# jinryan/RangeCLIP

Hardware: NVIDIA B200
Metric: pixel_text_infonce_fwd_bwd_throughput (higher is better)
Workload: dtype bf16

## Files before the change

rangeclip_b200/csrc/infonce_ts.cu:

```cuda
#include "infonce_pair.cuh"

namespace rc {
using namespace umma;

namespace ts {
using namespace cta_pair;

constexpr int kThreads = 640;
constexpr int kXStages = 6;
constexpr int kTStages = 3;
constexpr int kEpiBufs = 4;
constexpr int kEpiAhead = 2;
constexpr int kEpiBufBytes = 2048;
constexpr int kTmemCols = 512;
constexpr int kSlotCols = 256;
constexpr int kColAcc = 128, kAccCols = 64;
constexpr int kDxLead = 2;
constexpr int kRegsCtl = 48, kRegsSoftmax = 120;

struct __align__(8) Bars {
  uint64_t xf[kXStages];
  uint64_t xfull[kXStages], xempty[kXStages];
  uint64_t tfull[kTStages], tempty[kTStages];
  uint64_t s_full[2], p_full[2];
  uint64_t acc_full[2][2], acc_empty[2][2];
  uint64_t sc_full[4];
  uint64_t ebar[8][kEpiBufs];
  uint32_t tmem_base, pad;
};

constexpr int kScaleBufs = 4;
constexpr int kOffT = kXStages * kStageBytes;
constexpr int kOffEpi = kOffT + kTStages * kStageBytes;
constexpr int kOffScale = kOffEpi + 8 * kEpiBufs * kEpiBufBytes;
constexpr int kOffXch = kOffScale + kScaleBufs * 128 * 4;
constexpr int kOffPart = kOffXch + 2 * 4 * 2 * 128 * 4;
constexpr int kOffAcc = kOffPart + 8 * 128 * 4;
constexpr int kOffBars = kOffAcc + 3 * 128 * 4;
constexpr int kSmemBytes = kOffBars + (int)sizeof(Bars);
static_assert(kSmemBytes <= 232448, "shared-memory budget of one SM (227 KB)");

struct Params : Tiling {};

template <int R, bool kKB>
__global__ void __cluster_dims__(2, 1, 1) __launch_bounds__(kThreads, 1)
infonce_ts_kernel(const __grid_constant__ CUtensorMap map_x_s,
                  const __grid_constant__ CUtensorMap map_t,
                  const __grid_constant__ CUtensorMap map_tt,
                  const __grid_constant__ CUtensorMap map_xe,
                  const __grid_constant__ CUtensorMap map_dx,
                  const Params prm) {
  extern __shared__ __align__(1024) uint8_t smem[];
  Bars* bars = reinterpret_cast<Bars*>(smem + kOffBars);
  float* sc_s = reinterpret_cast<float*>(smem + kOffScale);
  const int warp = threadIdx.x >> 5, lane = threadIdx.x & 31;
  const uint32_t rank = cluster_ctarank();
  const bool leader_cta = rank == 0;
  const int n_dchunks = prm.D / 64;
  const int n_blk = prm.D / 64;
  const int n_kchunks = prm.Kp / 64;
  const int n_clusters = gridDim.x / 2;
  const int cluster_id = blockIdx.x / 2;
  const int my_pairs = cluster_id < prm.n_pairs ? (prm.n_pairs - cluster_id + n_clusters - 1) / n_clusters : 0;

  if (threadIdx.x == 0) {
    tma_prefetch_desc(&map_x_s); tma_prefetch_desc(&map_t); tma_prefetch_desc(&map_tt);
    tma_prefetch_desc(&map_xe); tma_prefetch_desc(&map_dx);
    for (int i = 0; i < kXStages; ++i) { mbar_init(&bars->xf[i], 1); mbar_init(&bars->xfull[i], 2); mbar_init(&bars->xempty[i], 9); }
    for (int i = 0; i < kTStages; ++i) { mbar_init(&bars->tfull[i], 1); mbar_init(&bars->tempty[i], 1); }
    for (int sl = 0; sl < 2; ++sl) {
      mbar_init(&bars->s_full[sl], 1); mbar_init(&bars->p_full[sl], 16);
      for (int ab = 0; ab < 2; ++ab) { mbar_init(&bars->acc_full[sl][ab], 1); mbar_init(&bars->acc_empty[sl][ab], 16); }
    }
    for (int i = 0; i < kScaleBufs; ++i) mbar_init(&bars->sc_full[i], 4);
    for (int i = 0; i < 8; ++i)
      for (int j = 0; j < kEpiBufs; ++j) mbar_init(&bars->ebar[i][j], 1);
    fence_barrier_init();
  }
  if (warp == 2) tmem_alloc_2sm<kTmemCols>(&bars->tmem_base);
  tc_fence_before();
  cluster_sync();
  tc_fence_after();
  const uint32_t tmem = bars->tmem_base;
#ifdef RC_TIMING
  long long wt[16];
#pragma unroll
  for (int i = 0; i < 16; ++i) wt[i] = 0;
  const long long t_start = clock64();
#endif
  const uint32_t idesc_s = make_idesc_bf16(256, prm.Kp,  1,  0);
  const uint32_t idesc_d = make_idesc_bf16(256, kAccCols, 0, 0);
  auto pair_of = [&](int l) -> int { return cluster_id + l * n_clusters; };

  if (warp < 4) {
    asm volatile("setmaxnreg.dec.sync.aligned.u32 %0;" ::"n"(kRegsCtl));
    if (warp == 0 && lane == 0) {
      uint32_t it = 0;
      auto load_s = [&](int l) {
        load_text_s<kTStages>(prm, &map_t, smem + kOffT, bars->tfull, bars->tempty, it, 0, n_dchunks,
                              text_row0<kKB>(prm, pair_of(l)), rank RC_WT);
      };
      auto load_dx = [&](int l, int b0, int b1) {
        const int koff = text_row0<kKB>(prm, pair_of(l));
        for (int blk = b0; blk < b1; ++blk, ++it) {
          const int st = it % kTStages;
          RC_WAIT(mbar_wait, &bars->tempty[st], ((it / kTStages) & 1) ^ 1, 2);
          if ((prm.ablate & 256) && it >= (uint32_t)kTStages) {
            if (leader_cta) mbar_arrive(&bars->tfull[st]);
            continue;
          }
          if (leader_cta) mbar_arrive_expect_tx(&bars->tfull[st], 2 * n_kchunks * 4096);
          for (int kc = 0; kc < n_kchunks; ++kc)
            tma_load_2d_2sm(smem + kOffT + st * kStageBytes + kc * 4096, &map_tt, &bars->tfull[st], koff + kc * 64,
                            blk * 64 + (int)rank * 32);
        }
      };
      if (my_pairs > 0) load_s(0);
      for (int l = 0; l < my_pairs; ++l) {
        load_dx(l, 0, kDxLead);
        if (l + 1 < my_pairs) load_s(l + 1);
        load_dx(l, kDxLead, n_blk);
      }
    } else if (warp == 3 && lane == 0) {
      uint32_t xit = 0;
      const uint64_t pol_keep = l2_policy_evict_last();
      for (int l = 0; l < my_pairs; ++l)
        load_x_tile<kXStages, kKB, true>(prm, &map_x_s, smem, bars->xf, bars->xempty, xit, 2 * pair_of(l) + (int)rank, n_dchunks,
                                         pol_keep, 3 RC_WT);
    } else if (warp == 1 && leader_cta) {
      uint32_t it = 0, xit = 0;
      uint32_t acc_par = 0;
      const uint32_t smem_base = smem_u32(smem);
      const uint64_t dsc_x = desc_mnmajor_sw128(0, 8192);
      const uint64_t dsc_k = desc_kmajor_sw128(0);
      auto wait_acc_free = [&](int sl, int ab, int tag) {
        RC_WAIT(mbar_wait, &bars->acc_empty[sl][ab], ((acc_par >> (2 * sl + ab)) & 1u) ^ 1u, tag);
      };
      auto issue_s = [&](int l) {
        const int sl = l & 1;
        const uint32_t s_tmem = tmem + sl * kSlotCols;
        wait_acc_free(sl, 0, 7);
        wait_acc_free(sl, 1, 7);
        tc_fence_after();
        RC_EV(l, 0);
        for (int c = 0; c < n_dchunks; ++c, ++it, ++xit) {
          const int sa = xit % kXStages, sb_ = it % kTStages;
          RC_WAIT(mbar_wait, &bars->xfull[sa], (xit / kXStages) & 1, 5);
          RC_WAIT(mbar_wait, &bars->tfull[sb_], (it / kTStages) & 1, 6);
          tc_fence_after();
          const uint64_t xa = dsc_x + ((smem_base + sa * kStageBytes) >> 4);
          const uint64_t tb = dsc_k + ((smem_base + kOffT + sb_ * kStageBytes) >> 4);
          if (elect_one()) {
#pragma unroll
            for (int ks = 0; ks < 4; ++ks)
              mma_bf16_ss_2sm(s_tmem, xa + ((ks * 2048) >> 4), tb + ((ks * 32) >> 4), idesc_s, (c | ks) != 0);
            mma_commit_2sm(&bars->xempty[sa]);
            mma_commit_2sm(&bars->tempty[sb_]);
            if (c + 1 == n_dchunks) mma_commit_2sm(&bars->s_full[sl]);
          }
          __syncwarp();
        }
        RC_EV(l, 1);
      };
      auto issue_dx = [&](int l, int b0, int b1) {
        const int sl = l & 1;
        const uint32_t base = tmem + sl * kSlotCols;
        if (b0 == 0) {
          RC_WAIT(mbar_wait, &bars->p_full[sl], (l >> 1) & 1, 9);
          tc_fence_after();
          RC_EV(l, 2);
        }
        for (int blk = b0; blk < b1; ++blk, ++it) {
          const int ab = blk & 1;
          wait_acc_free(sl, ab, 4);
          if (blk < 8) RC_EV(l, 3 + blk);
          const int st = it % kTStages;
          RC_WAIT(mbar_wait, &bars->tfull[st], (it / kTStages) & 1, 8);
          tc_fence_after();
          const uint64_t sb = dsc_k + ((smem_base + kOffT + st * kStageBytes) >> 4);
          const uint32_t dcol = base + kColAcc + ab * kAccCols;
          if (elect_one()) {
            for (int kc = 0; kc < n_kchunks; ++kc) {
#pragma unroll
              for (int ks = 0; ks < 4; ++ks)
                mma_bf16_ts_2sm(dcol, base + (kc * 4 + ks) * 8, sb + ((kc * 4096 + ks * 32) >> 4), idesc_d, (kc | ks) != 0);
            }
            mma_commit_2sm(&bars->tempty[st]);
            mma_commit_2sm(&bars->acc_full[sl][ab]);
          }
          __syncwarp();
          acc_par ^= 1u << (2 * sl + ab);
        }
        if (b1 == n_blk) RC_EV(l, 11);
      };
      if (my_pairs > 0) issue_s(0);
      for (int l = 0; l < my_pairs; ++l) {
        issue_dx(l, 0, kDxLead);
        if (l + 1 < my_pairs) issue_s(l + 1);
        issue_dx(l, kDxLead, n_blk);
      }
    } else if (warp == 2 && lane == 0) {
      uint32_t xit = 0;
      for (int l = 0; l < my_pairs; ++l) relay_x_tile<kXStages, false>(n_dchunks, bars->xf, bars->xfull, xit, leader_cta, 10 RC_WT);
    }
  } else if (warp < 12) {
    asm volatile("setmaxnreg.inc.sync.aligned.u32 %0;" ::"n"(kRegsSoftmax));
    const int half = warp >= 8 ? 1 : 0;
    const int row = (warp & 3) * 32 + lane;
    const int Kh = prm.Kp >> 1;
    const int cb = half * Kh;
    const uint32_t lane_base = tmem + ((uint32_t)((warp & 3) * 32) << 16);
    float* xch_base = reinterpret_cast<float*>(smem + kOffXch);
    float* acc_s = reinterpret_cast<float*>(smem + kOffAcc) + row;
    if (half == 0) acc_s[0] = acc_s[128] = acc_s[256] = 0.f;
    float gscale, inv_wsum;
    grad_scales(prm, gscale, inv_wsum);
    const float coefb = gscale * inv_wsum;
    float nx_ok, nx_w;
    int nx_y;
    load_pixel_scalars<R>(prm, 0 < my_pairs, 2 * pair_of(0) + (int)rank, row, nx_ok, nx_w, nx_y);
    float* part_s = reinterpret_cast<float*>(smem + kOffPart);
    int ng, nr;
    norm_coords(ng, nr);
    uint32_t nit = 0;
    const bool use_bound = prm.inv_tau * (2.02f * kLog2e) < 100.f;
    const float ml_bound = prm.inv_tau * (1.01f * kLog2e);
    for (int l = 0; l < my_pairs; ++l) {
      const int sl = l & 1;
      const int tile = 2 * pair_of(l) + (int)rank;
      const bool tile_ok = tile < prm.n_tiles;
      const int b = tile_ok ? div_tiles(prm, tile) : 0;
      const int px = tile_ok ? (tile - b * prm.tiles_per_img) * kTilePx + row : 0;
      const bool valid = tile_ok && px < prm.HW;
      const int64_t m = (int64_t)b * prm.HW + px;
      const int Kt = (kKB && prm.kb > 0) ? min(256, prm.K - 256 * b) : prm.K;
      const float ok = nx_ok;
      const bool px_ok = ok != 0.f;
      const int yi = nx_y;
      const float wi = (R == 1 && (yi >= 0 || (kKB && prm.keep_w))) ? nx_w : 0.f;
      load_pixel_scalars<R>(prm, l + 1 < my_pairs, 2 * pair_of(l + 1) + (int)rank, row, nx_ok, nx_w, nx_y);
      float* xch = xch_base + (l & 1) * (4 * 2 * 128);
      const uint32_t trow = lane_base + sl * kSlotCols + cb;
      RC_T0(tnorm);
      const float inv_n_tile = norm_tile<kXStages>(smem, bars->xf, bars->xempty, nit, n_dchunks, part_s, warp, lane, row, ng, nr, false,
                                                   11 RC_WT);
      RC_TACC(1, tnorm);
      if (warp == 4) RC_EV(l, 12);
      const float inv_n = px_ok ? inv_n_tile : 0.f;
      const float zs = inv_n * prm.inv_tau;
      const float zl = zs * kLog2e;
      RC_WAIT(mbar_wait, &bars->s_full[sl], (l >> 1) & 1, 12);
      tc_fence_after();
      if (warp == 4) RC_EV(l, 13);
      RC_T0(texp);
      const float ml = use_bound ? ml_bound : row_max(trow, Kt, cb, Kh, xch, half, row, zl);
      uint32_t pk[64];
      float sy[R];
      float sum, sez;
      exp_pass<R>(trow, cb, Kh, Kt, yi, zl, ml, pk, sy, sum, sez);
      int yj[R];
      float wj[R];
      bool mine[R];
      float wtot, tz;
      gather_targets<R>(prm, yi, wi, ok, m, cb, Kh, sy, yj, wj, mine, wtot, tz);
      post_sums(xch, half, row, sum, sez, tz);
      RC_TACC(2, texp);
      if (warp == 4) RC_EV(l, 14);
      tc_fence_before();
      RC_T0(txch);
      named_bar_sync(2, 256);
      RC_TACC(13, txch);
      tc_fence_after();
      RC_T0(tpst);
      add_peer_sums(xch, half, row, sum, sez, tz);
      const float lse = row_lse<kKB>(prm, valid, px, m, half, ml, wtot, tz, zs, sum, acc_s[0], acc_s[128]);
      const float coef = coefb * wtot;
      const float inv_sum = 1.f / sum;
      const float rsv = p_scale(inv_n, prm.inv_tau, coef, inv_sum);
      if (half == 0) {
        const float cj = proj_coef(coef, coefb, sez, tz, zs, inv_sum);
        sc_s[(l & (kScaleBufs - 1)) * 128 + row] = -(inv_n * inv_n * cj);
        acc_s[256] -= cj;
        __syncwarp();
        if (lane == 0) mbar_arrive(&bars->sc_full[l & (kScaleBufs - 1)]);
      }
      {
        const uint32_t prow = lane_base + sl * kSlotCols + (cb >> 1);
        const uint32_t rs2 = pack_bf16x2(rsv, rsv);
        uint32_t g16[R];
        int grel[R];
#pragma unroll
        for (int j = 0; j < R; ++j) {
          grel[j] = -1;
          g16[j] = 0;
          if (mine[j]) {
            const float gv = target_g<R>(j, sy, yj, wj, wtot, sum, zl, ml, rsv);
            grel[j] = yj[j] - cb;
            g16[j] = (uint32_t)__bfloat16_as_ushort(__float2bfloat16_rn(gv));
          }
        }
#pragma unroll
        for (int c = 0; c < 4; ++c) {
          if (c * 32 < Kh) {
            uint32_t v[16];
#pragma unroll
            for (int i = 0; i < 16; ++i) v[i] = bf2_mul(pk[c * 16 + i], rs2);
#pragma unroll
            for (int j = 0; j < R; ++j) {
              if (grel[j] >= 0 && (grel[j] >> 5) == c) {
                const int jj = (grel[j] >> 1) & 15;
                const bool hi = grel[j] & 1;
#pragma unroll
                for (int i = 0; i < 16; ++i)
                  if (i == jj) v[i] = hi ? ((v[i] & 0xffffu) | (g16[j] << 16)) : ((v[i] & 0xffff0000u) | g16[j]);
              }
            }
            tmem_st_32x16(prow + c * 16, v);
          }
        }
        tmem_st_wait();
        tc_fence_before();
        arrive_leader_warp(leader_cta, &bars->p_full[sl]);
      }
      RC_TACC(3, tpst);
      if (warp == 4) RC_EV(l, 15);
      if (half == 0 && valid && prm.lse && !(kKB && prm.lse_in != nullptr)) prm.lse[m] = lse;
    }
    if (half == 0) add_sums<true>(prm, lane, acc_s[0], acc_s[128], acc_s[256]);
  } else {
    const int ew = warp - 12;
    const int q = warp & 3, h = ew >> 2;
    uint8_t* ebuf = smem + kOffEpi + ew * (kEpiBufs * kEpiBufBytes);
    uint64_t* ebar = &bars->ebar[ew][0];
    const int total = my_pairs * n_blk;
    const uint64_t pol_first = l2_policy_evict_first();
    struct Cursor { int l, u, px, bo, bx; };
    auto cursor_pair = [&](Cursor& cu) {
      int b, px0;
      tile_coords(prm, 2 * pair_of(cu.l) + (int)rank, b, px0);
      cu.px = px0 + q * 32;
      cu.bo = b;
      cu.bx = (kKB && prm.kb > 0) ? (b < prm.B ? 0 : 1) : b;
    };
    auto cursor_next = [&](Cursor& cu) {
      if (++cu.u == n_blk) { cu.u = 0; ++cu.l; cursor_pair(cu); }
    };
    Cursor cs{0, 0, 0, 0, 0}, cr{0, 0, 0, 0, 0};
    cursor_pair(cs);
    cursor_pair(cr);
    int s_req = 0;
    auto request_x = [&]() {
      const int bi = s_req % kEpiBufs;
      if (prm.ablate & 1) {
        mbar_arrive(&ebar[bi]);
        return;
      }
      mbar_arrive_expect_tx(&ebar[bi], kEpiBufBytes);
      tma_load_3d_hint(ebuf + bi * kEpiBufBytes, &map_xe, &ebar[bi], cr.px, cr.u * 64 + h * 32, cr.bx, pol_first);
    };
    for (; s_req < kEpiAhead && s_req < total; ++s_req) {
      if (lane == 0) request_x();
      cursor_next(cr);
    }
    const uint32_t moff = (uint32_t)((lane & 7) * 64 + ((((lane >> 3) ^ ((lane >> 1) & 3)) & 3) << 4));
    int s = 0;
    uint32_t acc_par = 0;
    for (int l = 0; l < my_pairs; ++l) {
      const int sl = l & 1;
      RC_WAIT(mbar_wait, &bars->sc_full[l & (kScaleBufs - 1)], (l >> 2) & 1, 14);
      uint32_t ncs2[4];
#pragma unroll
      for (int pb = 0; pb < 4; ++pb) {
        const float v = sc_s[(l & (kScaleBufs - 1)) * 128 + q * 32 + pb * 8 + (lane >> 2)];
        ncs2[pb] = pack_bf16x2(v, v);
      }
      const uint32_t tacc = tmem + ((uint32_t)(q * 32) << 16) + sl * kSlotCols + kColAcc + h * 32;
      for (int blk = 0; blk < n_blk; ++blk, ++s) {
        const int ab = blk & 1;
        RC_WAIT(mbar_wait, &bars->acc_full[sl][ab], (acc_par >> (2 * sl + ab)) & 1u, 15);
        acc_par ^= 1u << (2 * sl + ab);
        tc_fence_after();
        if (warp == 12 && blk < 8) RC_EV(l, 20 + 2 * blk);
        RC_T0(tld);
        uint32_t pa[4][4];
        {
          uint32_t r[16];
          tmem_ld_16x256b_x4(tacc + ab * kAccCols, r);
          tmem_ld_wait();
#pragma unroll
          for (int g = 0; g < 4; ++g) {
            pa[g][0] = pack_bf16x2(__uint_as_float(r[4 * g]), __uint_as_float(r[4 * g + 1]));
            pa[g][1] = pack_bf16x2(__uint_as_float(r[4 * g + 2]), __uint_as_float(r[4 * g + 3]));
          }
          tmem_ld_16x256b_x4(tacc + ab * kAccCols + (16u << 16), r);
          tmem_ld_wait();
#pragma unroll
          for (int g = 0; g < 4; ++g) {
            pa[g][2] = pack_bf16x2(__uint_as_float(r[4 * g]), __uint_as_float(r[4 * g + 1]));
            pa[g][3] = pack_bf16x2(__uint_as_float(r[4 * g + 2]), __uint_as_float(r[4 * g + 3]));
          }
        }
        tc_fence_before();
        arrive_leader_warp(leader_cta, &bars->acc_empty[sl][ab]);
        RC_TACC(3, tld);
        const int bi = s % kEpiBufs;
        RC_WAIT(mbar_wait, &ebar[bi], (s / kEpiBufs) & 1, 4);
        RC_T0(tmath);
        const uint32_t bx0 = smem_u32(ebuf + bi * kEpiBufBytes) + moff;
        uint32_t xm[4][4];
#pragma unroll
        for (int g = 0; g < 4; ++g) ldmatrix_x4_trans(bx0 + g * 512, xm[g]);
#pragma unroll
        for (int g = 0; g < 4; ++g) {
#pragma unroll
          for (int pb = 0; pb < 4; ++pb) xm[g][pb] = bf2_fma(ncs2[pb], xm[g][pb], pa[g][pb]);
          stmatrix_x4_trans(bx0 + g * 512, xm[g]);
        }
        fence_proxy_async_smem();
        __syncwarp();
        RC_TACC(2, tmath);
        if (lane == 0) {
          if (!(prm.ablate & 2)) {
            if (kKB && prm.acc_dx) tma_reduce_add_3d(&map_dx, ebuf + bi * kEpiBufBytes, cs.px, cs.u * 64 + h * 32, cs.bo);
            else tma_store_3d_hint(&map_dx, ebuf + bi * kEpiBufBytes, cs.px, cs.u * 64 + h * 32, cs.bo, pol_first);
            tma_store_commit();
          }
          if (s_req < total) {
            RC_T0(tsw);
            asm volatile("cp.async.bulk.wait_group.read %0;" ::"n"(kEpiBufs - kEpiAhead) : "memory");
            RC_TACC(5, tsw);
            request_x();
          }
        }
        cursor_next(cs);
        if (s_req < total) { cursor_next(cr); ++s_req; }
        __syncwarp();
        if (warp == 12 && blk < 8) RC_EV(l, 21 + 2 * blk);
      }
    }
    if (lane == 0) tma_store_wait_all0();
  }
#ifdef RC_TIMING
  if (prm.dbg != nullptr && blockIdx.x < 2 && lane == 0 && (warp <= 1 || warp == 3 || warp == 4 || warp == 12)) {
    wt[0] = clock64() - t_start;
    const int role = warp == 0 ? 0 : (warp == 1 ? 1 : (warp == 4 ? 2 : (warp == 12 ? 3 : 4)));
#pragma unroll
    for (int i = 0; i < 16; ++i) prm.dbg[(blockIdx.x * 5 + role) * 16 + i] = wt[i];
  }
#endif
  tc_fence_before();
  cluster_sync();
  if (warp == 2) {
    tc_fence_after();
    tmem_dealloc_2sm<kTmemCols>(tmem);
  }
}

}

int launch_infonce_ts(const InfoncePairArgs& a, cudaStream_t s) {
  using namespace ts;
  CUtensorMap m_xs, m_t, m_tt, m_xe, m_dx;
  int rcode;
  if ((rcode = make_operand_maps(a, 32, {"ts map_x_s", "ts map_t", "ts map_tt"}, &m_xs, &m_t, &m_tt))) return rcode;
  if ((rcode = make_xmap(&m_xe, a.xsrc, a, a.kb > 0 ? 1 : a.B, 32, 32, "ts map_xe"))) return rcode;
  if ((rcode = make_xmap(&m_dx, a.dx, a, a.B, 32, 32, "ts map_dx"))) return rcode;
  Params prm;
  int grid = 0;
  if ((rcode = fill_tiling(prm, a, &grid))) return rcode;
  auto launch = [&](auto kernel) -> int {
    cudaError_t e = cudaFuncSetAttribute(kernel, cudaFuncAttributeMaxDynamicSharedMemorySize, kSmemBytes);
    if (e != cudaSuccess) return fail(RC_ERR_CUDA, "rc_infonce_bf16(ts): smem opt-in: %s", cudaGetErrorString(e));
    kernel<<<grid, kThreads, kSmemBytes, s>>>(m_xs, m_t, m_tt, m_xe, m_dx, prm);
    return check_launch("rc_infonce_bf16(ts)");
  };
  if (a.rep == 4) return launch(infonce_ts_kernel<4, false>);
  if (launch_kblocked(a)) return launch(infonce_ts_kernel<1, true>);
  return launch(infonce_ts_kernel<1, false>);
}

}
```

rangeclip_b200/csrc/umma.cuh:

```cuda
#pragma once
#include <cuda.h>
#include <cuda_runtime.h>
#include <stdint.h>
#include <stdio.h>

namespace rc {
namespace umma {

__device__ __forceinline__ uint32_t smem_u32(const void* p) {
  return (uint32_t)__cvta_generic_to_shared(p);
}

__device__ __forceinline__ void mbar_init(uint64_t* bar, uint32_t count) {
  asm volatile("mbarrier.init.shared::cta.b64 [%0], %1;" ::"r"(smem_u32(bar)), "r"(count) : "memory");
}
__device__ __forceinline__ void fence_barrier_init() {
  asm volatile("fence.mbarrier_init.release.cluster;" ::: "memory");
}
__device__ __forceinline__ void mbar_arrive(uint64_t* bar) {
  asm volatile("mbarrier.arrive.shared::cta.b64 _, [%0];" ::"r"(smem_u32(bar)) : "memory");
}
__device__ __forceinline__ void mbar_arrive_n(uint64_t* bar, uint32_t count) {
  asm volatile("mbarrier.arrive.shared::cta.b64 _, [%0], %1;" ::"r"(smem_u32(bar)), "r"(count) : "memory");
}
__device__ __forceinline__ void mbar_arrive_expect_tx(uint64_t* bar, uint32_t bytes) {
  asm volatile("mbarrier.arrive.expect_tx.shared::cta.b64 _, [%0], %1;" ::"r"(smem_u32(bar)), "r"(bytes) : "memory");
}
constexpr uint32_t kSuspendHintNs = 200000u;
__device__ __forceinline__ bool mbar_try_wait(uint64_t* bar, uint32_t parity) {
  uint32_t ok;
  asm volatile(
      "{\n\t.reg .pred p;\n\t"
      "mbarrier.try_wait.parity.shared::cta.b64 p, [%1], %2, %3;\n\t"
      "selp.u32 %0, 1, 0, p;\n\t}"
      : "=r"(ok)
      : "r"(smem_u32(bar)), "r"(parity), "r"(kSuspendHintNs)
      : "memory");
  return ok != 0;
}
__device__ __forceinline__ void mbar_wait(uint64_t* bar, uint32_t parity, int tag) {
#ifdef RC_BRINGUP
  if (mbar_try_wait(bar, parity)) return;
  const long long t0 = clock64();
  while (!mbar_try_wait(bar, parity)) {
    if (clock64() - t0 > 4000000000LL) {
      printf("rangeclip_b200: mbarrier timeout tag=%d block=%d thread=%d parity=%u\n", tag, (int)blockIdx.x,
             (int)threadIdx.x, parity);
      __trap();
    }
  }
#else
  (void)tag;
  while (!mbar_try_wait(bar, parity)) {}
#endif
}

__device__ __forceinline__ void fence_proxy_async_smem() {
  asm volatile("fence.proxy.async.shared::cta;" ::: "memory");
}
__device__ __forceinline__ void tc_fence_before() { asm volatile("tcgen05.fence::before_thread_sync;" ::: "memory"); }
__device__ __forceinline__ void tc_fence_after() { asm volatile("tcgen05.fence::after_thread_sync;" ::: "memory"); }
__device__ __forceinline__ void named_bar_sync(int id, int threads) {
  asm volatile("bar.sync %0, %1;" ::"r"(id), "r"(threads) : "memory");
}
__device__ __forceinline__ bool elect_one() {
  uint32_t pred;
  asm volatile(
      "{\n\t.reg .pred p;\n\t"
      "elect.sync _|p, 0xffffffff;\n\t"
      "selp.u32 %0, 1, 0, p;\n\t}"
      : "=r"(pred));
  return pred != 0;
}

__device__ __forceinline__ void tma_prefetch_desc(const CUtensorMap* m) {
  asm volatile("prefetch.tensormap [%0];" ::"l"(reinterpret_cast<uint64_t>(m)) : "memory");
}
__device__ __forceinline__ void tma_load_2d(void* dst, const CUtensorMap* m, uint64_t* bar, int c0, int c1) {
  asm volatile(
      "cp.async.bulk.tensor.2d.shared::cluster.global.mbarrier::complete_tx::bytes [%0], [%1, {%3, %4}], [%2];" ::"r"(
          smem_u32(dst)),
      "l"(reinterpret_cast<uint64_t>(m)), "r"(smem_u32(bar)), "r"(c0), "r"(c1)
      : "memory");
}
__device__ __forceinline__ void tma_load_3d(void* dst, const CUtensorMap* m, uint64_t* bar, int c0, int c1, int c2) {
  asm volatile(
      "cp.async.bulk.tensor.3d.shared::cluster.global.mbarrier::complete_tx::bytes [%0], [%1, {%3, %4, %5}], [%2];" ::"r"(
          smem_u32(dst)),
      "l"(reinterpret_cast<uint64_t>(m)), "r"(smem_u32(bar)), "r"(c0), "r"(c1), "r"(c2)
      : "memory");
}
__device__ __forceinline__ void tma_load_3d_hint(void* dst, const CUtensorMap* m, uint64_t* bar, int c0, int c1, int c2, uint64_t pol);
__device__ __forceinline__ uint64_t l2_policy_evict_first() {
  uint64_t p;
  asm volatile("createpolicy.fractional.L2::evict_first.b64 %0, 1.0;" : "=l"(p));
  return p;
}
__device__ __forceinline__ uint64_t l2_policy_evict_last() {
  uint64_t p;
  asm volatile("createpolicy.fractional.L2::evict_last.b64 %0, 1.0;" : "=l"(p));
  return p;
}
__device__ __forceinline__ void tma_load_3d_hint(void* dst, const CUtensorMap* m, uint64_t* bar, int c0, int c1, int c2, uint64_t pol) {
  asm volatile(
      "cp.async.bulk.tensor.3d.shared::cluster.global.mbarrier::complete_tx::bytes.L2::cache_hint [%0], [%1, {%3, %4, %5}], [%2], %6;" ::"r"(
          smem_u32(dst)),
      "l"(reinterpret_cast<uint64_t>(m)), "r"(smem_u32(bar)), "r"(c0), "r"(c1), "r"(c2), "l"(pol)
      : "memory");
}
__device__ __forceinline__ void tma_load_3d_2sm_hint(void* dst, const CUtensorMap* m, uint64_t* bar, int c0, int c1, int c2,
                                                     uint64_t pol) {
  asm volatile(
      "cp.async.bulk.tensor.3d.cta_group::2.shared::cluster.global.mbarrier::complete_tx::bytes.L2::cache_hint [%0], [%1, {%3, %4, %5}], [%2], %6;" ::"r"(
          smem_u32(dst)),
      "l"(reinterpret_cast<uint64_t>(m)), "r"(smem_u32(bar) & 0xFEFFFFFFu), "r"(c0), "r"(c1), "r"(c2), "l"(pol)
      : "memory");
}
__device__ __forceinline__ void tma_store_3d_hint(const CUtensorMap* m, const void* src, int c0, int c1, int c2, uint64_t pol) {
  asm volatile("cp.async.bulk.tensor.3d.global.shared::cta.bulk_group.L2::cache_hint [%0, {%2, %3, %4}], [%1], %5;" ::"l"(
                   reinterpret_cast<uint64_t>(m)),
               "r"(smem_u32(src)), "r"(c0), "r"(c1), "r"(c2), "l"(pol)
               : "memory");
}
__device__ __forceinline__ void tma_reduce_add_3d(const CUtensorMap* m, const void* src, int c0, int c1, int c2) {
  asm volatile("cp.reduce.async.bulk.tensor.3d.global.shared::cta.add.tile.bulk_group [%0, {%2, %3, %4}], [%1];" ::"l"(
                   reinterpret_cast<uint64_t>(m)),
               "r"(smem_u32(src)), "r"(c0), "r"(c1), "r"(c2)
               : "memory");
}
__device__ __forceinline__ void tma_prefetch_3d(const CUtensorMap* m, int c0, int c1, int c2) {
  asm volatile("cp.async.bulk.prefetch.tensor.3d.L2.global.tile [%0, {%1, %2, %3}];" ::"l"(reinterpret_cast<uint64_t>(m)), "r"(c0),
               "r"(c1), "r"(c2)
               : "memory");
}
__device__ __forceinline__ void tma_store_3d(const CUtensorMap* m, const void* src, int c0, int c1, int c2) {
  asm volatile("cp.async.bulk.tensor.3d.global.shared::cta.bulk_group [%0, {%2, %3, %4}], [%1];" ::"l"(
                   reinterpret_cast<uint64_t>(m)),
               "r"(smem_u32(src)), "r"(c0), "r"(c1), "r"(c2)
               : "memory");
}
__device__ __forceinline__ void tma_store_commit() { asm volatile("cp.async.bulk.commit_group;" ::: "memory"); }
__device__ __forceinline__ void tma_store_wait_read0() { asm volatile("cp.async.bulk.wait_group.read 0;" ::: "memory"); }
__device__ __forceinline__ void tma_store_wait_all0() { asm volatile("cp.async.bulk.wait_group 0;" ::: "memory"); }
__device__ __forceinline__ void tma_store_wait_read0_keep1() { asm volatile("cp.async.bulk.wait_group.read 1;" ::: "memory"); }

template <int kCols>
__device__ __forceinline__ void tmem_alloc(uint32_t* dst_smem) {
  asm volatile("tcgen05.alloc.cta_group::1.sync.aligned.shared::cta.b32 [%0], %1;" ::"r"(smem_u32(dst_smem)), "n"(kCols)
               : "memory");
  asm volatile("tcgen05.relinquish_alloc_permit.cta_group::1.sync.aligned;" ::: "memory");
}
template <int kCols>
__device__ __forceinline__ void tmem_dealloc(uint32_t taddr) {
  asm volatile("tcgen05.dealloc.cta_group::1.sync.aligned.b32 %0, %1;" ::"r"(taddr), "n"(kCols) : "memory");
}
__device__ __forceinline__ void tmem_ld_32x32(uint32_t taddr, uint32_t (&r)[32]) {
  asm volatile(
      "tcgen05.ld.sync.aligned.32x32b.x32.b32 "
      "{%0, %1, %2, %3, %4, %5, %6, %7, %8, %9, %10, %11, %12, %13, %14, %15, "
      "%16, %17, %18, %19, %20, %21, %22, %23, %24, %25, %26, %27, %28, %29, %30, %31}, [%32];"
      : "=r"(r[0]), "=r"(r[1]), "=r"(r[2]), "=r"(r[3]), "=r"(r[4]), "=r"(r[5]), "=r"(r[6]), "=r"(r[7]), "=r"(r[8]),
        "=r"(r[9]), "=r"(r[10]), "=r"(r[11]), "=r"(r[12]), "=r"(r[13]), "=r"(r[14]), "=r"(r[15]), "=r"(r[16]),
        "=r"(r[17]), "=r"(r[18]), "=r"(r[19]), "=r"(r[20]), "=r"(r[21]), "=r"(r[22]), "=r"(r[23]), "=r"(r[24]),
        "=r"(r[25]), "=r"(r[26]), "=r"(r[27]), "=r"(r[28]), "=r"(r[29]), "=r"(r[30]), "=r"(r[31])
      : "r"(taddr)
      : "memory");
}
__device__ __forceinline__ void tmem_ld_32x16(uint32_t taddr, uint32_t (&r)[16]) {
  asm volatile(
      "tcgen05.ld.sync.aligned.32x32b.x16.b32 "
      "{%0, %1, %2, %3, %4, %5, %6, %7, %8, %9, %10, %11, %12, %13, %14, %15}, [%16];"
      : "=r"(r[0]), "=r"(r[1]), "=r"(r[2]), "=r"(r[3]), "=r"(r[4]), "=r"(r[5]), "=r"(r[6]), "=r"(r[7]), "=r"(r[8]),
        "=r"(r[9]), "=r"(r[10]), "=r"(r[11]), "=r"(r[12]), "=r"(r[13]), "=r"(r[14]), "=r"(r[15])
      : "r"(taddr)
      : "memory");
}
__device__ __forceinline__ void tmem_ld_16x256b_x4(uint32_t taddr, uint32_t (&r)[16]) {
  asm volatile(
      "tcgen05.ld.sync.aligned.16x256b.x4.b32 "
      "{%0, %1, %2, %3, %4, %5, %6, %7, %8, %9, %10, %11, %12, %13, %14, %15}, [%16];"
      : "=r"(r[0]), "=r"(r[1]), "=r"(r[2]), "=r"(r[3]), "=r"(r[4]), "=r"(r[5]), "=r"(r[6]), "=r"(r[7]), "=r"(r[8]),
        "=r"(r[9]), "=r"(r[10]), "=r"(r[11]), "=r"(r[12]), "=r"(r[13]), "=r"(r[14]), "=r"(r[15])
      : "r"(taddr)
      : "memory");
}
__device__ __forceinline__ void ldmatrix_x4_trans(uint32_t saddr, uint32_t (&r)[4]) {
  asm volatile("ldmatrix.sync.aligned.m8n8.x4.trans.shared.b16 {%0, %1, %2, %3}, [%4];"
               : "=r"(r[0]), "=r"(r[1]), "=r"(r[2]), "=r"(r[3])
               : "r"(saddr)
               : "memory");
}
__device__ __forceinline__ void stmatrix_x4_trans(uint32_t saddr, const uint32_t (&r)[4]) {
  asm volatile("stmatrix.sync.aligned.m8n8.x4.trans.shared.b16 [%0], {%1, %2, %3, %4};" ::"r"(saddr), "r"(r[0]), "r"(r[1]),
               "r"(r[2]), "r"(r[3])
               : "memory");
}
__device__ __forceinline__ void tmem_st_32x16(uint32_t taddr, const uint32_t (&r)[16]) {
  asm volatile(
      "tcgen05.st.sync.aligned.32x32b.x16.b32 [%0], "
      "{%1, %2, %3, %4, %5, %6, %7, %8, %9, %10, %11, %12, %13, %14, %15, %16};" ::"r"(taddr),
      "r"(r[0]), "r"(r[1]), "r"(r[2]), "r"(r[3]), "r"(r[4]), "r"(r[5]), "r"(r[6]), "r"(r[7]), "r"(r[8]), "r"(r[9]), "r"(r[10]),
      "r"(r[11]), "r"(r[12]), "r"(r[13]), "r"(r[14]), "r"(r[15])
      : "memory");
}
__device__ __forceinline__ void tmem_st_wait() { asm volatile("tcgen05.wait::st.sync.aligned;" ::: "memory"); }
__device__ __forceinline__ void tmem_ld_wait() { asm volatile("tcgen05.wait::ld.sync.aligned;" ::: "memory"); }
__device__ __forceinline__ void tmem_ld_wait32(uint32_t (&r)[32]) {
  asm volatile("tcgen05.wait::ld.sync.aligned;"
               : "+r"(r[0]), "+r"(r[1]), "+r"(r[2]), "+r"(r[3]), "+r"(r[4]), "+r"(r[5]), "+r"(r[6]), "+r"(r[7]), "+r"(r[8]),
                 "+r"(r[9]), "+r"(r[10]), "+r"(r[11]), "+r"(r[12]), "+r"(r[13]), "+r"(r[14]), "+r"(r[15]), "+r"(r[16]),
                 "+r"(r[17]), "+r"(r[18]), "+r"(r[19]), "+r"(r[20]), "+r"(r[21]), "+r"(r[22]), "+r"(r[23]), "+r"(r[24]),
                 "+r"(r[25]), "+r"(r[26]), "+r"(r[27]), "+r"(r[28]), "+r"(r[29]), "+r"(r[30]), "+r"(r[31])
               :
               : "memory");
}

__host__ __device__ constexpr uint64_t make_smem_desc_sw128(uint32_t smem_addr, uint32_t lbo_bytes, uint32_t sbo_bytes) {
  return (uint64_t)((smem_addr >> 4) & 0x3FFF) | ((uint64_t)((lbo_bytes >> 4) & 0x3FFF) << 16) |
         ((uint64_t)((sbo_bytes >> 4) & 0x3FFF) << 32) | (1ull << 46) | (2ull << 61);
}
__device__ __forceinline__ uint64_t desc_kmajor_sw128(uint32_t smem_addr) {
  return make_smem_desc_sw128(smem_addr, 16, 1024);
}
__device__ __forceinline__ uint64_t desc_mnmajor_sw128(uint32_t smem_addr, uint32_t mn_group_stride_bytes) {
  return make_smem_desc_sw128(smem_addr, mn_group_stride_bytes, 1024);
}
__host__ __device__ constexpr uint32_t make_idesc_bf16(int M, int N, int a_mn_major, int b_mn_major) {
  return (1u << 4) | (1u << 7) | (1u << 10) | ((uint32_t)a_mn_major << 15) | ((uint32_t)b_mn_major << 16) |
         ((uint32_t)(N >> 3) << 17) | ((uint32_t)(M >> 4) << 24);
}
__device__ __forceinline__ void mma_bf16_ss(uint32_t d_tmem, uint64_t a_desc, uint64_t b_desc, uint32_t idesc,
                                            uint32_t accumulate) {
  asm volatile(
      "{\n\t.reg .pred p;\n\t"
      "setp.ne.b32 p, %4, 0;\n\t"
      "tcgen05.mma.cta_group::1.kind::f16 [%0], %1, %2, %3, p;\n\t}" ::"r"(d_tmem),
      "l"(a_desc), "l"(b_desc), "r"(idesc), "r"(accumulate)
      : "memory");
}
__device__ __forceinline__ void mma_commit(uint64_t* bar) {
  asm volatile("tcgen05.commit.cta_group::1.mbarrier::arrive::one.shared::cluster.b64 [%0];" ::"r"(smem_u32(bar))
               : "memory");
}


__device__ __forceinline__ uint32_t cluster_ctarank() {
  uint32_t r;
  asm volatile("mov.u32 %0, %%cluster_ctarank;" : "=r"(r));
  return r;
}
__device__ __forceinline__ void cluster_sync() {
  asm volatile("barrier.cluster.arrive.aligned;" ::: "memory");
  asm volatile("barrier.cluster.wait.aligned;" ::: "memory");
}
__device__ __forceinline__ uint32_t map_to_cta(const void* p, uint32_t rank) {
  uint32_t r;
  asm volatile("mapa.shared::cluster.u32 %0, %1, %2;" : "=r"(r) : "r"(smem_u32(p)), "r"(rank));
  return r;
}
__device__ __forceinline__ void mbar_arrive_remote(uint32_t cluster_addr) {
  asm volatile("mbarrier.arrive.shared::cluster.b64 _, [%0];" ::"r"(cluster_addr) : "memory");
}
__device__ __forceinline__ void st_async_remote_v2(uint32_t cluster_addr, uint32_t a, uint32_t b, uint32_t cluster_mbar) {
  asm volatile("st.async.weak.shared::cluster.mbarrier::complete_tx::bytes.v2.b32 [%0], {%1, %2}, [%3];" ::"r"(cluster_addr),
               "r"(a), "r"(b), "r"(cluster_mbar)
               : "memory");
}
__device__ __forceinline__ void st_async_remote_b32(uint32_t cluster_addr, uint32_t a, uint32_t cluster_mbar) {
  asm volatile("st.async.weak.shared::cluster.mbarrier::complete_tx::bytes.b32 [%0], %1, [%2];" ::"r"(cluster_addr), "r"(a),
               "r"(cluster_mbar)
               : "memory");
}
__device__ __forceinline__ uint32_t bf2_mul(uint32_t a, uint32_t b) {
  uint32_t d;
  asm("mul.rn.bf16x2 %0, %1, %2;" : "=r"(d) : "r"(a), "r"(b));
  return d;
}
__device__ __forceinline__ uint32_t bf2_fma(uint32_t a, uint32_t b, uint32_t c) {
  uint32_t d;
  asm("fma.rn.bf16x2 %0, %1, %2, %3;" : "=r"(d) : "r"(a), "r"(b), "r"(c));
  return d;
}
__device__ __forceinline__ bool mbar_try_wait_cluster(uint64_t* bar, uint32_t parity) {
  uint32_t ok;
  asm volatile(
      "{\n\t.reg .pred p;\n\t"
      "mbarrier.try_wait.parity.acquire.cluster.shared::cta.b64 p, [%1], %2, %3;\n\t"
      "selp.u32 %0, 1, 0, p;\n\t}"
      : "=r"(ok)
      : "r"(smem_u32(bar)), "r"(parity), "r"(kSuspendHintNs)
      : "memory");
  return ok != 0;
}
__device__ __forceinline__ void mbar_wait_cluster(uint64_t* bar, uint32_t parity, int tag) {
#ifdef RC_BRINGUP
  if (mbar_try_wait_cluster(bar, parity)) return;
  const long long t0 = clock64();
  while (!mbar_try_wait_cluster(bar, parity)) {
    if (clock64() - t0 > 4000000000LL) {
      printf("rangeclip_b200: cluster mbarrier timeout tag=%d block=%d thread=%d parity=%u\n", tag, (int)blockIdx.x,
             (int)threadIdx.x, parity);
      __trap();
    }
  }
#else
  (void)tag;
  while (!mbar_try_wait_cluster(bar, parity)) {}
#endif
}
constexpr uint32_t kPeerBitMask = 0xFEFFFFFFu;
__device__ __forceinline__ void tma_load_2d_2sm(void* dst, const CUtensorMap* m, uint64_t* bar, int c0, int c1) {
  asm volatile(
      "cp.async.bulk.tensor.2d.cta_group::2.shared::cluster.global.mbarrier::complete_tx::bytes [%0], [%1, {%3, %4}], [%2];" ::"r"(
          smem_u32(dst)),
      "l"(reinterpret_cast<uint64_t>(m)), "r"(smem_u32(bar) & kPeerBitMask), "r"(c0), "r"(c1)
      : "memory");
}
__device__ __forceinline__ void tma_load_3d_2sm(void* dst, const CUtensorMap* m, uint64_t* bar, int c0, int c1, int c2) {
  asm volatile(
      "cp.async.bulk.tensor.3d.cta_group::2.shared::cluster.global.mbarrier::complete_tx::bytes [%0], [%1, {%3, %4, %5}], [%2];" ::"r"(
          smem_u32(dst)),
      "l"(reinterpret_cast<uint64_t>(m)), "r"(smem_u32(bar) & kPeerBitMask), "r"(c0), "r"(c1), "r"(c2)
      : "memory");
}
template <int kCols>
__device__ __forceinline__ void tmem_alloc_2sm(uint32_t* dst_smem) {
  asm volatile("tcgen05.alloc.cta_group::2.sync.aligned.shared::cta.b32 [%0], %1;" ::"r"(smem_u32(dst_smem)), "n"(kCols)
               : "memory");
  asm volatile("tcgen05.relinquish_alloc_permit.cta_group::2.sync.aligned;" ::: "memory");
}
template <int kCols>
__device__ __forceinline__ void tmem_dealloc_2sm(uint32_t taddr) {
  asm volatile("tcgen05.dealloc.cta_group::2.sync.aligned.b32 %0, %1;" ::"r"(taddr), "n"(kCols) : "memory");
}
__device__ __forceinline__ void mma_bf16_ss_2sm(uint32_t d_tmem, uint64_t a_desc, uint64_t b_desc, uint32_t idesc,
                                                uint32_t accumulate) {
  asm volatile(
      "{\n\t.reg .pred p;\n\t"
      "setp.ne.b32 p, %4, 0;\n\t"
      "tcgen05.mma.cta_group::2.kind::f16 [%0], %1, %2, %3, p;\n\t}" ::"r"(d_tmem),
      "l"(a_desc), "l"(b_desc), "r"(idesc), "r"(accumulate)
      : "memory");
}
__device__ __forceinline__ void mma_bf16_ts_2sm(uint32_t d_tmem, uint32_t a_tmem, uint64_t b_desc, uint32_t idesc,
                                                uint32_t accumulate) {
  asm volatile(
      "{\n\t.reg .pred p;\n\t"
      "setp.ne.b32 p, %4, 0;\n\t"
      "tcgen05.mma.cta_group::2.kind::f16 [%0], [%1], %2, %3, p;\n\t}" ::"r"(d_tmem),
      "r"(a_tmem), "l"(b_desc), "r"(idesc), "r"(accumulate)
      : "memory");
}
__device__ __forceinline__ void mma_commit_2sm(uint64_t* bar) {
  asm volatile(
      "tcgen05.commit.cta_group::2.mbarrier::arrive::one.shared::cluster.multicast::cluster.b64 [%0], %1;" ::"r"(
          smem_u32(bar)),
      "h"((uint16_t)3)
      : "memory");
}

}

typedef CUresult (*PFN_encodeTiled)(CUtensorMap*, CUtensorMapDataType, cuuint32_t, void*, const cuuint64_t*,
                                    const cuuint64_t*, const cuuint32_t*, const cuuint32_t*, CUtensorMapInterleave,
                                    CUtensorMapSwizzle, CUtensorMapL2promotion, CUtensorMapFloatOOBfill);
PFN_encodeTiled get_encode_tiled();

int make_tmap_bf16(CUtensorMap* out, const void* base, int rank, const uint64_t* dims, const uint64_t* strides_bytes,
                   const uint32_t* box, const char* what);

}
```

Baseline: 1845.

## Pair epilogue warps on 64-pixel TMA boxes with split load/store roles

Epilogue warps are now paired so that each pair shares one 64-pixel-wide swizzled buffer (4 KB) instead of each warp owning a 32-pixel box. One warp of each pair issues the input prefetch loads and the other issues the dx stores, synchronised through a named barrier, which halves the number of TMA operations. The two TMEM loads are batched before a single wait, and the S/dx issue order is factored into a shared helper with an optional S split (kSParts=1, so the schedule is unchanged). The cost is an extra 64-thread barrier per block and more coupling between warps.

```diff
diff --git a/rangeclip_b200/csrc/infonce_ts.cu b/rangeclip_b200/csrc/infonce_ts.cu
--- a/rangeclip_b200/csrc/infonce_ts.cu
+++ b/rangeclip_b200/csrc/infonce_ts.cu
@@ -11,11 +11,13 @@
 constexpr int kTStages = 3;
 constexpr int kEpiBufs = 4;
 constexpr int kEpiAhead = 2;
-constexpr int kEpiBufBytes = 2048;
+constexpr int kEpiBufBytes = 4096;
+constexpr int kEpiPairs = 4;
 constexpr int kTmemCols = 512;
 constexpr int kSlotCols = 256;
 constexpr int kColAcc = 128, kAccCols = 64;
 constexpr int kDxLead = 2;
+constexpr int kSParts = 1;
 constexpr int kRegsCtl = 48, kRegsSoftmax = 120;
 
 struct __align__(8) Bars {
@@ -25,14 +27,15 @@
   uint64_t s_full[2], p_full[2];
   uint64_t acc_full[2][2], acc_empty[2][2];
   uint64_t sc_full[4];
-  uint64_t ebar[8][kEpiBufs];
+  uint64_t ebar[kEpiPairs][kEpiBufs];
   uint32_t tmem_base, pad;
 };
 
 constexpr int kScaleBufs = 4;
 constexpr int kOffT = kXStages * kStageBytes;
 constexpr int kOffEpi = kOffT + kTStages * kStageBytes;
-constexpr int kOffScale = kOffEpi + 8 * kEpiBufs * kEpiBufBytes;
+constexpr int kOffScale = kOffEpi + kEpiPairs * kEpiBufs * kEpiBufBytes;
+static_assert(kOffEpi % 1024 == 0 && kEpiBufBytes % 1024 == 0, "128-byte swizzled epilogue boxes are 1024-byte aligned");
 constexpr int kOffXch = kOffScale + kScaleBufs * 128 * 4;
 constexpr int kOffPart = kOffXch + 2 * 4 * 2 * 128 * 4;
 constexpr int kOffAcc = kOffPart + 8 * 128 * 4;
@@ -41,6 +44,24 @@
 static_assert(kSmemBytes <= 232448, "shared-memory budget of one SM (227 KB)");
 
 struct Params : Tiling {};
+
+template <class FS, class FD>
+__device__ __forceinline__ void walk_issue_order(int my_pairs, int n_dchunks, int n_blk, FS&& on_s, FD&& on_dx) {
+  if (my_pairs > 0) on_s(0, 0, n_dchunks);
+  for (int l = 0; l < my_pairs; ++l) {
+    int b = 0;
+    if (l + 1 < my_pairs) {
+#pragma unroll
+      for (int p = 0; p < kSParts; ++p) {
+        const int b1 = min(b + kDxLead, n_blk);
+        on_dx(l, b, b1);
+        b = b1;
+        on_s(l + 1, p * n_dchunks / kSParts, (p + 1) * n_dchunks / kSParts);
+      }
+    }
+    on_dx(l, b, n_blk);
+  }
+}
 
 template <int R, bool kKB>
 __global__ void __cluster_dims__(2, 1, 1) __launch_bounds__(kThreads, 1)
@@ -73,7 +94,7 @@
       for (int ab = 0; ab < 2; ++ab) { mbar_init(&bars->acc_full[sl][ab], 1); mbar_init(&bars->acc_empty[sl][ab], 16); }
     }
     for (int i = 0; i < kScaleBufs; ++i) mbar_init(&bars->sc_full[i], 4);
-    for (int i = 0; i < 8; ++i)
+    for (int i = 0; i < kEpiPairs; ++i)
       for (int j = 0; j < kEpiBufs; ++j) mbar_init(&bars->ebar[i][j], 1);
     fence_barrier_init();
   }
@@ -96,8 +117,8 @@
     asm volatile("setmaxnreg.dec.sync.aligned.u32 %0;" ::"n"(kRegsCtl));
     if (warp == 0 && lane == 0) {
       uint32_t it = 0;
-      auto load_s = [&](int l) {
-        load_text_s<kTStages>(prm, &map_t, smem + kOffT, bars->tfull, bars->tempty, it, 0, n_dchunks,
+      auto load_s = [&](int l, int c0, int c1) {
+        load_text_s<kTStages>(prm, &map_t, smem + kOffT, bars->tfull, bars->tempty, it, c0, c1,
                               text_row0<kKB>(prm, pair_of(l)), rank RC_WT);
       };
       auto load_dx = [&](int l, int b0, int b1) {
@@ -115,12 +136,7 @@
                             blk * 64 + (int)rank * 32);
         }
       };
-      if (my_pairs > 0) load_s(0);
-      for (int l = 0; l < my_pairs; ++l) {
-        load_dx(l, 0, kDxLead);
-        if (l + 1 < my_pairs) load_s(l + 1);
-        load_dx(l, kDxLead, n_blk);
-      }
+      walk_issue_order(my_pairs, n_dchunks, n_blk, load_s, load_dx);
     } else if (warp == 3 && lane == 0) {
       uint32_t xit = 0;
       const uint64_t pol_keep = l2_policy_evict_last();
@@ -136,14 +152,16 @@
       auto wait_acc_free = [&](int sl, int ab, int tag) {
         RC_WAIT(mbar_wait, &bars->acc_empty[sl][ab], ((acc_par >> (2 * sl + ab)) & 1u) ^ 1u, tag);
       };
-      auto issue_s = [&](int l) {
+      auto issue_s = [&](int l, int c0, int c1) {
         const int sl = l & 1;
         const uint32_t s_tmem = tmem + sl * kSlotCols;
-        wait_acc_free(sl, 0, 7);
-        wait_acc_free(sl, 1, 7);
-        tc_fence_after();
-        RC_EV(l, 0);
-        for (int c = 0; c < n_dchunks; ++c, ++it, ++xit) {
+        if (c0 == 0) {
+          wait_acc_free(sl, 0, 7);
+          wait_acc_free(sl, 1, 7);
+          tc_fence_after();
+          RC_EV(l, 0);
+        }
+        for (int c = c0; c < c1; ++c, ++it, ++xit) {
           const int sa = xit % kXStages, sb_ = it % kTStages;
           RC_WAIT(mbar_wait, &bars->xfull[sa], (xit / kXStages) & 1, 5);
           RC_WAIT(mbar_wait, &bars->tfull[sb_], (it / kTStages) & 1, 6);
@@ -160,7 +178,7 @@
           }
           __syncwarp();
         }
-        RC_EV(l, 1);
+        if (c1 == n_dchunks) RC_EV(l, 1);
       };
       auto issue_dx = [&](int l, int b0, int b1) {
         const int sl = l & 1;
@@ -193,12 +211,7 @@
         }
         if (b1 == n_blk) RC_EV(l, 11);
       };
-      if (my_pairs > 0) issue_s(0);
-      for (int l = 0; l < my_pairs; ++l) {
-        issue_dx(l, 0, kDxLead);
-        if (l + 1 < my_pairs) issue_s(l + 1);
-        issue_dx(l, kDxLead, n_blk);
-      }
+      walk_issue_order(my_pairs, n_dchunks, n_blk, issue_s, issue_dx);
     } else if (warp == 2 && lane == 0) {
       uint32_t xit = 0;
       for (int l = 0; l < my_pairs; ++l) relay_x_tile<kXStages, false>(n_dchunks, bars->xf, bars->xfull, xit, leader_cta, 10 RC_WT);
@@ -330,24 +343,25 @@
   } else {
     const int ew = warp - 12;
     const int q = warp & 3, h = ew >> 2;
-    uint8_t* ebuf = smem + kOffEpi + ew * (kEpiBufs * kEpiBufBytes);
-    uint64_t* ebar = &bars->ebar[ew][0];
+    const int ep = ew >> 1;
+    const bool storer = (q & 1) == 0;
+    uint8_t* ebuf = smem + kOffEpi + ep * (kEpiBufs * kEpiBufBytes);
+    uint64_t* ebar = &bars->ebar[ep][0];
     const int total = my_pairs * n_blk;
     const uint64_t pol_first = l2_policy_evict_first();
     struct Cursor { int l, u, px, bo, bx; };
     auto cursor_pair = [&](Cursor& cu) {
       int b, px0;
       tile_coords(prm, 2 * pair_of(cu.l) + (int)rank, b, px0);
-      cu.px = px0 + q * 32;
+      cu.px = px0 + (q >> 1) * 64;
       cu.bo = b;
       cu.bx = (kKB && prm.kb > 0) ? (b < prm.B ? 0 : 1) : b;
     };
     auto cursor_next = [&](Cursor& cu) {
       if (++cu.u == n_blk) { cu.u = 0; ++cu.l; cursor_pair(cu); }
     };
-    Cursor cs{0, 0, 0, 0, 0}, cr{0, 0, 0, 0, 0};
-    cursor_pair(cs);
-    cursor_pair(cr);
+    Cursor cu{0, 0, 0, 0, 0};
+    cursor_pair(cu);
     int s_req = 0;
     auto request_x = [&]() {
       const int bi = s_req % kEpiBufs;
@@ -356,13 +370,15 @@
         return;
       }
       mbar_arrive_expect_tx(&ebar[bi], kEpiBufBytes);
-      tma_load_3d_hint(ebuf + bi * kEpiBufBytes, &map_xe, &ebar[bi], cr.px, cr.u * 64 + h * 32, cr.bx, pol_first);
+      tma_load_3d_hint(ebuf + bi * kEpiBufBytes, &map_xe, &ebar[bi], cu.px, cu.u * 64 + h * 32, cu.bx, pol_first);
     };
-    for (; s_req < kEpiAhead && s_req < total; ++s_req) {
-      if (lane == 0) request_x();
-      cursor_next(cr);
+    if (!storer) {
+      for (; s_req < kEpiAhead && s_req < total; ++s_req) {
+        if (lane == 0) request_x();
+        cursor_next(cu);
+      }
     }
-    const uint32_t moff = (uint32_t)((lane & 7) * 64 + ((((lane >> 3) ^ ((lane >> 1) & 3)) & 3) << 4));
+    const uint32_t moff = (uint32_t)((lane & 7) * 128 + (((((q & 1) << 2) | (lane >> 3)) ^ (lane & 7)) << 4));
     int s = 0;
     uint32_t acc_par = 0;
     for (int l = 0; l < my_pairs; ++l) {
@@ -384,20 +400,16 @@
         RC_T0(tld);
         uint32_t pa[4][4];
         {
-          uint32_t r[16];
-          tmem_ld_16x256b_x4(tacc + ab * kAccCols, r);
-          tmem_ld_wait();
+          uint32_t r[32];
+          tmem_ld_16x256b_x4_both(tacc + ab * kAccCols, r);
+          tmem_ld_wait32(r);
 #pragma unroll
           for (int g = 0; g < 4; ++g) {
-            pa[g][0] = pack_bf16x2(__uint_as_float(r[4 * g]), __uint_as_float(r[4 * g + 1]));
-            pa[g][1] = pack_bf16x2(__uint_as_float(r[4 * g + 2]), __uint_as_float(r[4 * g + 3]));
-          }
-          tmem_ld_16x256b_x4(tacc + ab * kAccCols + (16u << 16), r);
-          tmem_ld_wait();
-#pragma unroll
-          for (int g = 0; g < 4; ++g) {
-            pa[g][2] = pack_bf16x2(__uint_as_float(r[4 * g]), __uint_as_float(r[4 * g + 1]));
-            pa[g][3] = pack_bf16x2(__uint_as_float(r[4 * g + 2]), __uint_as_float(r[4 * g + 3]));
+#pragma unroll
+            for (int hh = 0; hh < 2; ++hh) {
+              pa[g][2 * hh] = pack_bf16x2(__uint_as_float(r[16 * hh + 4 * g]), __uint_as_float(r[16 * hh + 4 * g + 1]));
+              pa[g][2 * hh + 1] = pack_bf16x2(__uint_as_float(r[16 * hh + 4 * g + 2]), __uint_as_float(r[16 * hh + 4 * g + 3]));
+            }
           }
         }
         tc_fence_before();
@@ -409,31 +421,38 @@
         const uint32_t bx0 = smem_u32(ebuf + bi * kEpiBufBytes) + moff;
         uint32_t xm[4][4];
 #pragma unroll
-        for (int g = 0; g < 4; ++g) ldmatrix_x4_trans(bx0 + g * 512, xm[g]);
+        for (int g = 0; g < 4; ++g) ldmatrix_x4_trans(bx0 + g * 1024, xm[g]);
 #pragma unroll
         for (int g = 0; g < 4; ++g) {
 #pragma unroll
           for (int pb = 0; pb < 4; ++pb) xm[g][pb] = bf2_fma(ncs2[pb], xm[g][pb], pa[g][pb]);
-          stmatrix_x4_trans(bx0 + g * 512, xm[g]);
+          stmatrix_x4_trans(bx0 + g * 1024, xm[g]);
         }
         fence_proxy_async_smem();
-        __syncwarp();
         RC_TACC(2, tmath);
+        RC_T0(tsw);
+        if (storer && lane == 0) asm volatile("cp.async.bulk.wait_group.read %0;" ::"n"(kEpiBufs - kEpiAhead - 1) : "memory");
+        RC_TACC(5, tsw);
+        RC_T0(tsy);
+        named_bar_sync(8 + ep, 64);
+        RC_TACC(8, tsy);
         if (lane == 0) {
-          if (!(prm.ablate & 2)) {
-            if (kKB && prm.acc_dx) tma_reduce_add_3d(&map_dx, ebuf + bi * kEpiBufBytes, cs.px, cs.u * 64 + h * 32, cs.bo);
-            else tma_store_3d_hint(&map_dx, ebuf + bi * kEpiBufBytes, cs.px, cs.u * 64 + h * 32, cs.bo, pol_first);
-            tma_store_commit();
-          }
-          if (s_req < total) {
-            RC_T0(tsw);
-            asm volatile("cp.async.bulk.wait_group.read %0;" ::"n"(kEpiBufs - kEpiAhead) : "memory");
-            RC_TACC(5, tsw);
+          if (storer) {
+            if (!(prm.ablate & 2)) {
+              RC_T0(tst);
+              if (kKB && prm.acc_dx) tma_reduce_add_3d(&map_dx, ebuf + bi * kEpiBufBytes, cu.px, cu.u * 64 + h * 32, cu.bo);
+              else tma_store_3d_hint(&map_dx, ebuf + bi * kEpiBufBytes, cu.px, cu.u * 64 + h * 32, cu.bo, pol_first);
+              tma_store_commit();
+              RC_TACC(6, tst);
+            }
+          } else if (s_req < total) {
+            RC_T0(trq);
             request_x();
-          }
-        }
-        cursor_next(cs);
-        if (s_req < total) { cursor_next(cr); ++s_req; }
+            RC_TACC(7, trq);
+          }
+        }
+        if (storer) cursor_next(cu);
+        else if (s_req < total) { cursor_next(cu); ++s_req; }
         __syncwarp();
         if (warp == 12 && blk < 8) RC_EV(l, 21 + 2 * blk);
       }
@@ -441,11 +460,11 @@
     if (lane == 0) tma_store_wait_all0();
   }
 #ifdef RC_TIMING
-  if (prm.dbg != nullptr && blockIdx.x < 2 && lane == 0 && (warp <= 1 || warp == 3 || warp == 4 || warp == 12)) {
+  if (prm.dbg != nullptr && blockIdx.x < 2 && lane == 0 && (warp <= 1 || warp == 3 || warp == 4 || warp == 12 || warp == 13)) {
     wt[0] = clock64() - t_start;
-    const int role = warp == 0 ? 0 : (warp == 1 ? 1 : (warp == 4 ? 2 : (warp == 12 ? 3 : 4)));
-#pragma unroll
-    for (int i = 0; i < 16; ++i) prm.dbg[(blockIdx.x * 5 + role) * 16 + i] = wt[i];
+    const int role = warp == 0 ? 0 : (warp == 1 ? 1 : (warp == 4 ? 2 : (warp == 12 ? 3 : (warp == 13 ? 5 : 4))));
+#pragma unroll
+    for (int i = 0; i < 16; ++i) prm.dbg[(blockIdx.x * 6 + role) * 16 + i] = wt[i];
   }
 #endif
   tc_fence_before();
@@ -463,8 +482,8 @@
   CUtensorMap m_xs, m_t, m_tt, m_xe, m_dx;
   int rcode;
   if ((rcode = make_operand_maps(a, 32, {"ts map_x_s", "ts map_t", "ts map_tt"}, &m_xs, &m_t, &m_tt))) return rcode;
-  if ((rcode = make_xmap(&m_xe, a.xsrc, a, a.kb > 0 ? 1 : a.B, 32, 32, "ts map_xe"))) return rcode;
-  if ((rcode = make_xmap(&m_dx, a.dx, a, a.B, 32, 32, "ts map_dx"))) return rcode;
+  if ((rcode = make_xmap(&m_xe, a.xsrc, a, a.kb > 0 ? 1 : a.B, 64, 32, "ts map_xe"))) return rcode;
+  if ((rcode = make_xmap(&m_dx, a.dx, a, a.B, 64, 32, "ts map_dx"))) return rcode;
   Params prm;
   int grid = 0;
   if ((rcode = fill_tiling(prm, a, &grid))) return rcode;
diff --git a/rangeclip_b200/csrc/umma.cuh b/rangeclip_b200/csrc/umma.cuh
--- a/rangeclip_b200/csrc/umma.cuh
+++ b/rangeclip_b200/csrc/umma.cuh
@@ -184,6 +184,10 @@
       : "r"(taddr)
       : "memory");
 }
+__device__ __forceinline__ void tmem_ld_16x256b_x4_both(uint32_t taddr, uint32_t (&r)[32]) {
+  tmem_ld_16x256b_x4(taddr, *reinterpret_cast<uint32_t(*)[16]>(&r[0]));
+  tmem_ld_16x256b_x4(taddr + (16u << 16), *reinterpret_cast<uint32_t(*)[16]>(&r[16]));
+}
 __device__ __forceinline__ void ldmatrix_x4_trans(uint32_t saddr, uint32_t (&r)[4]) {
   asm volatile("ldmatrix.sync.aligned.m8n8.x4.trans.shared.b16 {%0, %1, %2, %3}, [%4];"
                : "=r"(r[0]), "=r"(r[1]), "=r"(r[2]), "=r"(r[3])
```

New measurement: 1898 (median of 6 runs). 2.9% higher.
